# rsasaki0109/lidarslam_ros2

Hardware: AMD Instinct MI355X
Metric: scan registrations/sec (30k-pt scan vs 10-frame submap) (higher is better)
Workload: dtype f32; 1 GPU; cfg2: single NDT align(), 30000-pt VLP-32 scan (vg 0.2) vs 10-frame submap (vg 0.1), ndt_resolution 5.0, DIRECT7, max_iterations 30, transformation_epsilon 0; 1018 different scans (stream of 64); target_points=661519, voxels_valid=643, derivative_passes_last_scan=242, parallelism=1 registration stream per GPU x1, collective=none (one rank)

## Files before the change

### include/lidarslam_reg.h

```cpp
#ifndef LIDARSLAM_REG_H
#define LIDARSLAM_REG_H

#include <stddef.h>
#include <stdint.h>

#ifdef __cplusplus
extern "C" {
#endif

typedef struct lsr_handle_s* lsr_handle;

typedef enum lsr_status {
  LSR_OK = 0,
  LSR_ERR_INVALID_ARGUMENT = -1,
  LSR_ERR_NO_DEVICE = -2,
  LSR_ERR_HIP = -3,
  LSR_ERR_NO_TARGET = -4,
  LSR_ERR_NO_SOURCE = -5,
  LSR_ERR_NOT_IMPLEMENTED = -6,
  LSR_ERR_INDEX_OVERFLOW = -7,
  LSR_ERR_TOO_FEW_POINTS = -8
} lsr_status;

typedef enum lsr_method { LSR_METHOD_NDT = 0, LSR_METHOD_GICP = 1 } lsr_method;
// ... 6 lines not shown
  LSR_STEP_SIZE = 2,
  LSR_OUTLIER_RATIO = 3,
  LSR_MAX_CORRESPONDENCE_DISTANCE = 4,
  LSR_ROTATION_EPSILON = 5,
  LSR_EUCLIDEAN_FITNESS_EPSILON = 6,
  LSR_GICP_EPSILON = 7,
  LSR_MAP_ASSEMBLY_MS = 8,
  LSR_MAX_ITERATIONS = 32,
  LSR_NEIGHBORHOOD = 33,
  LSR_NUM_THREADS = 34,
  LSR_K_CORRESPONDENCES = 35,
  LSR_MAX_INNER_ITERATIONS = 36,
  LSR_RANSAC_ITERATIONS = 37,
  LSR_HESSIAN_D1_SIGN = 38,
  LSR_PROFILE = 39,
  LSR_NDT_WORKGROUP = 40,
  LSR_NDT_TABLE_MODE = 41,
  LSR_GRID_BUILDER = 42,
  LSR_WAIT_MODE = 43,
  LSR_NDT_QUAD = 44,
  LSR_VOXEL_FILTER_FORM = 46,
  LSR_NDT_SPLIT = 47,
  LSR_TARGET_PREPARED = 48,
  LSR_MAP_ASSEMBLY_FORM = 49
} lsr_key;

typedef struct lsr_result {
  int32_t converged;
  int32_t iterations;
  double score;
  int32_t n_evaluations;
  int32_t n_correspondences;
  double gpu_ms;
} lsr_result;

typedef struct lsr_profile {
  double deriv_ms_total;
  int64_t deriv_launches;
  int64_t deriv_points;
  int64_t deriv_pairs;
} lsr_profile;

const char* lsr_version(void);
const char* lsr_status_string(int status);
const char* lsr_last_error(void);
int lsr_device_count(int* count);

int lsr_create(int method, int device_id, void* stream, lsr_handle* out);
int lsr_destroy(lsr_handle h);

int lsr_set_f64(lsr_handle h, int key, double value);
int lsr_set_i32(lsr_handle h, int key, int value);
int lsr_get_f64(lsr_handle h, int key, double* value);
int lsr_get_i32(lsr_handle h, int key, int* value);

int lsr_set_input_target(lsr_handle h, const void* pts, size_t stride_bytes, size_t n);
int lsr_set_input_target_device(lsr_handle h, const void* dev_pts, size_t stride_bytes, size_t n);
int lsr_set_input_target_batch(lsr_handle* handles, int count, const void* const* clouds, const size_t* counts,
                               size_t stride_bytes, int on_device);
int lsr_wait_stream(lsr_handle h, void* producer_stream);
int lsr_set_input_target_frames(lsr_handle h, int n_frames, const void* const* frames, const size_t* counts, size_t stride_bytes,
                                const float* poses16, int on_device);
int lsr_set_input_target_frames_filtered(lsr_handle h, int n_frames, const void* const* frames, const size_t* counts,
// ... 128 lines not shown
```

### lidarslam_ros2_amd/_capi.py

```python
from __future__ import annotations

import ctypes as C
import os

_HERE = os.path.dirname(os.path.abspath(__file__))
LIB_PATH = os.path.join(_HERE, os.environ.get("LSR_LIB_NAME", "liblidarslam_reg.so"))

OK = 0
METHOD_NDT, METHOD_GICP = 0, 1
KDTREE, DIRECT26, DIRECT7, DIRECT1 = 0, 1, 2, 3
(RESOLUTION, TRANSFORMATION_EPSILON, STEP_SIZE, OUTLIER_RATIO, MAX_CORRESPONDENCE_DISTANCE, ROTATION_EPSILON,
 EUCLIDEAN_FITNESS_EPSILON, GICP_EPSILON, MAP_ASSEMBLY_MS) = range(9)
(MAX_ITERATIONS, NEIGHBORHOOD, NUM_THREADS, K_CORRESPONDENCES, MAX_INNER_ITERATIONS, RANSAC_ITERATIONS,
 HESSIAN_D1_SIGN, PROFILE, NDT_WORKGROUP, NDT_TABLE_MODE, GRID_BUILDER, WAIT_MODE, NDT_QUAD, _UNASSIGNED_45, VOXEL_FILTER_FORM, NDT_SPLIT, TARGET_PREPARED,
 MAP_ASSEMBLY_FORM) = range(32, 50)

EXPORTED_SYMBOLS = [
    "lsr_version", "lsr_status_string", "lsr_last_error", "lsr_device_count", "lsr_create", "lsr_destroy",
    "lsr_set_f64", "lsr_set_i32", "lsr_get_f64", "lsr_get_i32", "lsr_set_input_target", "lsr_set_input_target_device",
    "lsr_set_input_target_frames", "lsr_set_input_source", "lsr_set_input_source_device", "lsr_set_input_source_filtered", "lsr_set_input_source_frontend", "lsr_voxel_grid_filter",
    "lsr_share_target", "lsr_wait_stream", "lsr_align", "lsr_align_batch",
    "lsr_get_final_transformation", "lsr_has_converged", "lsr_get_fitness_score", "lsr_search_loop", "lsr_ndt_grid_info",
    "lsr_ndt_grid_dump", "lsr_ndt_grid_centroids", "lsr_ndt_derivatives", "lsr_ndt_derivatives_pairs", "lsr_gicp_covariances", "lsr_nearest_neighbors", "lsr_get_profile",
    "lsr_debug_angle_tables", "lsr_set_input_source_pc2", "lsr_get_source_pc2", "lsr_voxel_grid_filter_pc2", "lsr_shard_range", "lsr_comm_unique_id", "lsr_comm_create", "lsr_comm_destroy", "lsr_align_batch_sharded",
    "lsr_shard_plan", "lsr_align_batch_planned", "lsr_align_fitness_batch",
    "lsr_set_input_target_batch", "lsr_set_input_source_batch", "lsr_get_fitness_score_batch", "lsr_set_input_target_bcast", "lsr_get_source_pc2_device",
    "lsr_comm_all_gather_records", "lsr_set_input_target_frames_filtered", "lsr_prepare_target", "lsr_gicp_linearize",
    "lsr_imu_reset", "lsr_imu_push", "lsr_imu_receive", "lsr_imu_info", "lsr_deskew_pc2", "lsr_deskew_trace",
    "lsr_assemble_map",
]


class Result(C.Structure):
    _fields_ = [("converged", C.c_int32), ("iterations", C.c_int32), ("score", C.c_double),
                ("n_evaluations", C.c_int32), ("n_correspondences", C.c_int32), ("gpu_ms", C.c_double)]


class Profile(C.Structure):
    _fields_ = [("deriv_ms_total", C.c_double), ("deriv_launches", C.c_int64), ("deriv_points", C.c_int64),
                ("deriv_pairs", C.c_int64)]


class SubMap(C.Structure):
    _fields_ = [("position", C.c_double * 3), ("orientation", C.c_double * 4), ("distance", C.c_double),
                ("cloud", C.c_void_p), ("n_points", C.c_size_t)]


class LoopParams(C.Structure):
    _fields_ = [("threshold_loop_closure_score", C.c_double), ("distance_loop_closure", C.c_double),
                ("range_of_searching_loop_closure", C.c_double), ("search_submap_num", C.c_int),
                ("voxel_leaf_size", C.c_float), ("top_k", C.c_int), ("reserved", C.c_int)]


class LoopEdge(C.Structure):
    _fields_ = [("id_from", C.c_int), ("id_to", C.c_int), ("accepted", C.c_int), ("converged", C.c_int),
                ("iterations", C.c_int), ("n_target_points", C.c_int), ("candidate_distance", C.c_double),
                ("fitness_score", C.c_double), ("relative_pose", C.c_double * 16), ("final_transformation", C.c_float * 16)]


class Pc2Layout(C.Structure):
    _fields_ = [("point_step", C.c_uint32), ("offset_x", C.c_uint32), ("offset_y", C.c_uint32), ("offset_z", C.c_uint32),
                ("offset_intensity", C.c_int32)]

# ... 115 lines not shown
```

### lidarslam_ros2_amd/csrc/capi.hip

```cpp
#include <algorithm>
#include <chrono>
#include <functional>
#include <limits>
#include <cmath>
#include <cstdlib>
#include <mutex>
#include <numeric>
#include <thread>

#include "handle.hpp"

namespace lsr {
static thread_local std::string g_last_error;
void set_last_error(const std::string& s) { g_last_error = s; }
}

using namespace lsr;

namespace {

#define LSR_CHECK_HANDLE(h)                      \
  if (!(h)) {                                    \
    set_last_error("null handle");               \
    return LSR_ERR_INVALID_ARGUMENT;             \
// ... 569 lines not shown
  if (eager && !st) st = eager_dispatch(true);
  if (eager) {
    (void)hipEventRecord(lead->side_ev, lead->side_stream);
    for (int b = 0; b < B; b++) {
      if (!eager_sent[b]) continue;
      double v = 0;
      const int fst = nn_fitness_end(hs[b]->scratch, lead->side_stream, &v);
      if (fst && !st) st = fst;
      if (!fst) fitness_out[b] = v;
    }
  }
  if (prefetched || eager) {
    if (hipEventSynchronize(lead->side_ev) != hipSuccess && !st) { set_last_error("side-stream work of the candidate set failed"); st = LSR_ERR_HIP; }
    if (st && prefetched) for (int b = 0; b < B; b++) if (hs[b]->target) hs[b]->target->has_hash = false;
  }
  if (st) return st;
  const double ms = std::chrono::duration<double, std::milli>(std::chrono::steady_clock::now() - t0).count();
  const NdtMailbox* M = lead->mailbox.p;
  if (lead->profile) {
    LSR_HIP(hipEventRecord(lead->ev1, lead->stream));
    LSR_HIP(hipEventSynchronize(lead->ev1));
    float ev_ms = 0.f;
    LSR_HIP(hipEventElapsedTime(&ev_ms, lead->ev0, lead->ev1));
    int passes = 0;
    lead->prof.deriv_pairs = 0;
    for (int b = 0; b < B; b++) {
      passes = std::max(passes, M[b].n_passes);
      lead->prof.deriv_pairs += (int64_t)M[b].last_pairs;
    }
    lead->prof.deriv_ms_total += ev_ms;
    lead->prof.deriv_launches += passes;
    lead->prof.deriv_points += (int64_t)passes * pts;
  }
  for (int b = 0; b < B; b++) {
    lsr_handle h = hs[b];
    std::memcpy(h->final_T, M[b].final_T, sizeof(float) * 16);
    h->converged = M[b].converged;
    if (finals) std::memcpy(finals + 16 * b, M[b].final_T, sizeof(float) * 16);
    if (results) {
      results[b].converged = M[b].converged;
      results[b].iterations = M[b].nr_iterations;
      results[b].score = M[b].trans_probability;
      results[b].n_evaluations = M[b].n_evals;
      results[b].n_correspondences = (int)M[b].last_pairs;
      results[b].gpu_ms = ms;
    }
  }
  return LSR_OK;
}

}

extern "C" {

// ... 154 lines not shown
      if (v < 3 || v > GICP_MAX_K) { set_last_error("k_correspondences out of range"); return LSR_ERR_INVALID_ARGUMENT; }
      h->gicp.k = v; h->source_cov_valid = false; if (h->target) h->target->has_cov = false; return LSR_OK;
    case LSR_MAX_INNER_ITERATIONS: h->gicp.max_inner = v; return LSR_OK;
    case LSR_RANSAC_ITERATIONS: h->ransac_iterations = v; return LSR_OK;
    case LSR_HESSIAN_D1_SIGN: h->ndt.d1_sign = (v >= 0) ? 1 : -1; return LSR_OK;
    case LSR_PROFILE: h->profile = v ? 1 : 0; return LSR_OK;
    case LSR_NDT_WORKGROUP:
      if (v == 256) {
        static bool warned = false;
        if (!warned) { warned = true; fprintf(stderr, "[lidarslam_reg] LSR_NDT_WORKGROUP = 256 is a geometry of an earlier kernel: using the automatic choice (0)\n"); }
        h->ndt_threads = 0; return LSR_OK;
      }
      if (v != 0 && v != 64 && v != 128 && v != 512 && v != 1024) { set_last_error("NDT workgroup key must be 0 (auto), 64 / 128 (quad kernel: points) or 512 / 1024 (lane kernel: threads)"); return LSR_ERR_INVALID_ARGUMENT; }
      h->ndt_threads = v; return LSR_OK;
    case LSR_NDT_TABLE_MODE:
      if (v < -1 || v > 2) { set_last_error("NDT table mode must be in -1 .. 2: -1 (auto), 0 dense, 1 compact, 2 LDS"); return LSR_ERR_INVALID_ARGUMENT; }
      h->ndt_table_mode = v; return LSR_OK;
    case LSR_NDT_QUAD:
      if (v < -1 || v > 1) { set_last_error("NDT quad mode must be -1 (auto), 0 or 1"); return LSR_ERR_INVALID_ARGUMENT; }
      h->ndt_quad = v; return LSR_OK;
    case LSR_NDT_SPLIT:
      if (v < -1 || v > 1) { set_last_error("NDT split mode must be -1 (auto), 0 or 1"); return LSR_ERR_INVALID_ARGUMENT; }
      h->ndt_split = v; return LSR_OK;
    case LSR_GRID_BUILDER:
      if (v < 0 || v > 1) { set_last_error("grid builder must be 0 (auto) or 1 (radix-sort builder)"); return LSR_ERR_INVALID_ARGUMENT; }
      h->scratch.force_sort_path = (v == 1);
      if (h->target) h->target->has_grid = h->target->has_centroids = false;
      return LSR_OK;
    case LSR_WAIT_MODE:
      if (v < 0 || v > 2) { set_last_error("wait mode must be 0 (spin), 1 (yield) or 2 (sleep)"); return LSR_ERR_INVALID_ARGUMENT; }
      h->scratch.wait_mode = v; return LSR_OK;
    default: set_last_error("unknown i32 key"); return LSR_ERR_INVALID_ARGUMENT;
  }
}

int lsr_get_i32(lsr_handle h, int key, int* v) {
  LSR_CHECK_HANDLE(h);
  if (!v) return LSR_ERR_INVALID_ARGUMENT;
  switch (key) {
    case LSR_MAX_ITERATIONS: *v = (h->method == LSR_METHOD_NDT) ? h->ndt.max_iterations : h->gicp.max_iterations; return LSR_OK;
    case LSR_NEIGHBORHOOD: *v = h->ndt.neighborhood; return LSR_OK;
    case LSR_NUM_THREADS: *v = h->num_threads; return LSR_OK;
    case LSR_K_CORRESPONDENCES: *v = h->gicp.k; return LSR_OK;
    case LSR_MAX_INNER_ITERATIONS: *v = h->gicp.max_inner; return LSR_OK;
    case LSR_RANSAC_ITERATIONS: *v = h->ransac_iterations; return LSR_OK;
    case LSR_HESSIAN_D1_SIGN: *v = h->ndt.d1_sign; return LSR_OK;
    case LSR_PROFILE: *v = h->profile; return LSR_OK;
    case LSR_NDT_WORKGROUP: *v = h->ndt_threads; return LSR_OK;
    case LSR_NDT_TABLE_MODE: *v = h->ndt_table_mode; return LSR_OK;
    case LSR_NDT_QUAD: *v = h->ndt_quad; return LSR_OK;
    case LSR_NDT_SPLIT: *v = h->ndt_split; return LSR_OK;
    case LSR_GRID_BUILDER: *v = h->scratch.force_sort_path ? 1 : 0; return LSR_OK;
    case LSR_WAIT_MODE: *v = h->scratch.wait_mode; return LSR_OK;
    case LSR_VOXEL_FILTER_FORM: *v = h->scratch.vg_form; return LSR_OK;
    case LSR_MAP_ASSEMBLY_FORM: *v = h->map_form; return LSR_OK;
    case LSR_TARGET_PREPARED:
      if (h->method == LSR_METHOD_GICP) *v = gicp_target_prepared(h) ? 1 : 0;
      else *v = (h->target && h->target->n > 0 && h->target->has_grid && h->target->grid_leaf == (float)h->ndt.resolution &&
                 (h->ndt.neighborhood != LSR_KDTREE || h->target->has_centroids || h->target->grid.ncells == 0)) ? 1 : 0;
      return LSR_OK;
    default: set_last_error("unknown i32 key"); return LSR_ERR_INVALID_ARGUMENT;
  }
}

static int set_target_impl(lsr_handle h, const void* pts, size_t stride, size_t n, bool on_device) {
  LSR_CHECK_HANDLE(h);
  if (h->method == LSR_METHOD_NDT) {
    lsr_handle one[1] = {h};
    const void* cloud[1] = {pts};
    const size_t count[1] = {n};
    return lsr_set_input_target_batch(one, 1, cloud, count, stride, on_device ? 1 : 0);
  }
  auto t = fresh_target(h);
  int st = upload_cloud(h, pts, stride, n, on_device, t->cloud);
// ... 1020 lines not shown
  if (grad) for (int i = 0; i < 6; i++) grad[i] = S.g[i];
  if (hess) for (int i = 0; i < 36; i++) hess[i] = compute_hessian ? S.H[i] : 0.0;
  if (pairs) *pairs = S.last_pairs;
  return LSR_OK;
}

int lsr_gicp_covariances(lsr_handle h, int which, double* cov) {
  LSR_CHECK_HANDLE(h);
  if (!cov) return LSR_ERR_INVALID_ARGUMENT;
  return gicp_get_covariances(h, which, cov);
}

int lsr_gicp_linearize(lsr_handle h, const float* guess16, const float* trans16, int use_seeds, float* out, int32_t* nn_idx,
                       int32_t* valid, double* M6, float* q, double* x6, float* T12, double* dR27, int32_t* m, double* sums28) {
  LSR_CHECK_HANDLE(h);
  if (h->method != LSR_METHOD_GICP) { set_last_error("lsr_gicp_linearize on an NDT object"); return LSR_ERR_INVALID_ARGUMENT; }
  const GicpLinearizeOut o{out, nn_idx, valid, M6, q, x6, T12, dR27, m, sums28};
  return gicp_linearize(h, guess16, trans16, use_seeds, o);
}

int lsr_get_profile(lsr_handle h, lsr_profile* out, int reset) {
  LSR_CHECK_HANDLE(h);
  if (out) *out = h->prof;
  if (reset) h->prof = lsr_profile{0, 0, 0, 0};
  return LSR_OK;
}

}
```

### lidarslam_ros2_amd/csrc/handle.hpp

```cpp
#pragma once
#include "common.hpp"
#include "deskew.hpp"
#include "gicp.hpp"
#include "ndt.hpp"
#include "nn.hpp"

namespace lsr {
struct StreamDep {
  hipEvent_t ev = nullptr;
  ~StreamDep() { if (ev) (void)hipEventDestroy(ev); }
};
}

struct lsr_handle_s {
  using NdtParamsHost = lsr::NdtParamsHost; using GicpParamsHost = lsr::GicpParamsHost; using TargetData = lsr::TargetData;
  using DeviceCloud = lsr::DeviceCloud; using HashGridDev = lsr::HashGridDev; using BuildScratch = lsr::BuildScratch;
  using NdtState = lsr::NdtState; using NdtProblem = lsr::NdtProblem; using GicpWorkspace = lsr::GicpWorkspace;
  template <typename T> using DevBuf = lsr::DevBuf<T>;
  template <typename T> using PinBuf = lsr::PinBuf<T>;
  int method = LSR_METHOD_NDT;
  int device = 0;
  hipStream_t stream = nullptr;
  bool own_stream = false;
  hipEvent_t ev0 = nullptr, ev1 = nullptr;
// ... 39 lines not shown
  const NdtState* h_state_dev = nullptr;
  const NdtProblem* h_prob_dev = nullptr;
  PinBuf<lsr::NdtMailbox> mailbox;
  lsr::NdtMailbox* d_mailbox = nullptr;
  unsigned int align_token = 0;
  DevBuf<float> d_T16;
  DevBuf<float> d_poses;
  DevBuf<lsr::FrameSlot> d_frames;
  PinBuf<lsr::FrameSlot> h_frames;
  DevBuf<lsr::MapSlot> d_map_slots;
  PinBuf<lsr::MapSlot> h_map_slots;
  DevBuf<unsigned char> map_out;
  int map_form = 0;
  double map_ms = 0.0;

  GicpWorkspace gicp_ws;

  lsr::DeskewState deskew;

  std::vector<std::unique_ptr<lsr_handle_s>> aux;

  float final_T[16] = {1, 0, 0, 0, 0, 1, 0, 0, 0, 0, 1, 0, 0, 0, 0, 1};
  int converged = 0;
  lsr_profile prof = {0, 0, 0, 0};
};
```

### lidarslam_ros2_amd/csrc/ndt.hip

```cpp
#include "ndt.hpp"

#include <cmath>
#include <cstdlib>
#include <type_traits>

#include "grid_device.hpp"
#include "ndt_point.hpp"
#include "sort.hpp"

namespace lsr {

namespace {

__host__ __device__ inline void angle_tables(const double* p, bool with_hessian, int d1_sign, float* jang, float* hang) {
  double cx, cy, cz, sx, sy, sz;
  if (fabs(p[3]) < 10e-5) { cx = 1.0; sx = 0.0; } else { cx = cos(p[3]); sx = sin(p[3]); }
  if (fabs(p[4]) < 10e-5) { cy = 1.0; sy = 0.0; } else { cy = cos(p[4]); sy = sin(p[4]); }
  if (fabs(p[5]) < 10e-5) { cz = 1.0; sz = 0.0; } else { cz = cos(p[5]); sz = sin(p[5]); }
  jang[0] = (float)(-sx * sz + cx * sy * cz); jang[1] = (float)(-sx * cz - cx * sy * sz); jang[2] = (float)(-cx * cy);
  jang[3] = (float)(cx * sz + sx * sy * cz);  jang[4] = (float)(cx * cz - sx * sy * sz);  jang[5] = (float)(-sx * cy);
  jang[6] = (float)(-sy * cz);                jang[7] = (float)(sy * sz);                 jang[8] = (float)(cy);
  jang[9] = (float)(sx * cy * cz);            jang[10] = (float)(-sx * cy * sz);          jang[11] = (float)(sx * sy);
  jang[12] = (float)(-cx * cy * cz);          jang[13] = (float)(cx * cy * sz);           jang[14] = (float)(-cx * sy);
  jang[15] = (float)(-cy * sz);               jang[16] = (float)(-cy * cz);               jang[17] = 0.f;
// ... 33 lines not shown
  float s1 = sinf(res[0]), c1 = cosf(res[0]);
  res[2] = atan2f(s1 * c(2, 0) - c1 * c(1, 0), c1 * c(1, 1) - s1 * c(2, 1));
  res[0] = -res[0]; res[1] = -res[1]; res[2] = -res[2];
}

}

void ndt_gauss_constants(double resolution, double outlier_ratio, double* d1, double* d2) {
  double c1 = 10 * (1 - outlier_ratio);
  double c2 = outlier_ratio / pow(resolution, 3);
  double d3 = -log(c2);
  *d1 = -log(c1 + c2) - d3;
  *d2 = -2 * log((-log(c1 * exp(-0.5) + c2) - d3) / *d1);
}

void ndt_fill_align_constants(NdtState& st, const NdtParamsHost& prm, int n_points) {
  ndt_gauss_constants(prm.resolution, prm.outlier_ratio, &st.d1, &st.d2);
  st.step_max = prm.step_size;
  st.step_min = prm.trans_eps / 2;
  st.eps = prm.trans_eps;
  st.max_iter = prm.max_iterations;
  st.n_points = n_points;
  st.d1_sign = prm.d1_sign;
}

void ndt_fill_initial_state(NdtState& st, const float* guess16 , const NdtParamsHost& prm, int n_points) {
  std::memset(&st, 0, sizeof(st));
  ndt_fill_align_constants(st, prm, n_points);
  float I16[16] = {1, 0, 0, 0, 0, 1, 0, 0, 0, 0, 1, 0, 0, 0, 0, 1};
  const float* G = guess16 ? guess16 : I16;
  std::memcpy(st.final_T, G, sizeof(I16));
  st.T[0] = G[0]; st.T[1] = G[4]; st.T[2] = G[8];  st.T[3] = G[12];
  st.T[4] = G[1]; st.T[5] = G[5]; st.T[6] = G[9];  st.T[7] = G[13];
  st.T[8] = G[2]; st.T[9] = G[6]; st.T[10] = G[10]; st.T[11] = G[14];
  float e[3];
  euler012_f(G, e);
  st.p[0] = G[12]; st.p[1] = G[13]; st.p[2] = G[14];
  st.p[3] = e[0]; st.p[4] = e[1]; st.p[5] = e[2];
  for (int i = 0; i < 6; i++) st.x_t[i] = st.p[i];
  angle_tables(st.p, true, st.d1_sign, st.jang, st.hang);
  st.want_hessian = 1;
  st.phase = PH_INIT;
  st.done = 0;
}

void ndt_fill_diag_state(NdtState& st, const double* p6, const float* T16, int compute_hessian, const NdtParamsHost& prm,
// ... 256 lines not shown
  } else if (lane == 6) {
    f[0] = 1.0;
    f[7] = 0.0;
  }
  wave_lds_fence();
  const bool with_hang = (mode & 2) != 0;
  if (lane < 24 || with_hang) {
    double val = angle_entry_value(ent_a, f);
    if (lane == 24 + 20 && S->d1_sign < 0) val = -val;
    if (lane < 24) S->jang[lane] = (float)val; else S->hang[lane - 24] = (float)val;
  }
  if (with_hang && lane < 8) S->hang[40 + lane] = (float)angle_entry_value(ent_b, f);
  if (lane == 63) {
    float* T = S->T;
    compose_R12(cs_f[0], cs_f[1], cs_f[2], cs_f[3], cs_f[4], cs_f[5], T);
    T[3] = (float)S->x_t[0]; T[7] = (float)S->x_t[1]; T[11] = (float)S->x_t[2];
    T12_to_colmajor16(T, S->final_T);
  }
  if (lane == 0) S->pad1 = 0;
  wave_lds_fence();
}

enum CtlNext : int { CTL_DONE = 0, CTL_NEWTON_BEGIN = 1, CTL_NEWTON_END = 2 };

__device__ __forceinline__ int ndt_controller_mt(LdsState* S, const LdsDouble* sums) {
  const double mu = 1.e-4, nu = 0.9;
  const int max_step_iterations = 10;
  double sv[8];
#pragma unroll
  for (int k = 0; k < 8; k++) sv[k] = sums[k];
  const int phase = S->phase;
  const bool had_hessian = S->want_hessian != 0;
  const int n_evals = S->n_evals + (phase == PH_MT_LAST ? 2 : 1);
  const int n_passes = S->n_passes + 1;
  if (phase == PH_INIT || phase == PH_MT_HESS || phase == PH_DIAG) {
    S->n_evals = n_evals;
    S->n_passes = n_passes;
    S->last_pairs = sv[7];
    if (phase != PH_MT_HESS) {
      S->score = sv[0];
#pragma unroll
      for (int i = 0; i < 6; i++) S->g[i] = sv[1 + i];
    }
    if (phase == PH_DIAG) {
      if (had_hessian) {
        double hu[21];
#pragma unroll
        for (int k = 0; k < 21; k++) hu[k] = sums[8 + k];
        int k = 0;
#pragma unroll
// ... 222 lines not shown
    unsigned long long* _r = (unsigned long long*)&g_lsr_timing[(810 + ((hess) ? 1 : 0)) * 32]; \
    atomicAdd(&_r[0], 1ull); atomicAdd(&_r[1], (unsigned long long)(_p_t1 - _p_t0)); atomicAdd(&_r[2], (unsigned long long)(_p_t2 - _p_t7)); \
    atomicAdd(&_r[3], (unsigned long long)(_t3 - _p_t2)); atomicAdd(&_r[4], (unsigned long long)(_c3 - _p_c0)); atomicAdd(&_r[5], (unsigned long long)(_t3 - _p_t0)); \
  }
#else
#define LSR_STAMP(k)
#define LSR_STAMP_T(k, t)
#define LSR_SPAN_BEGIN(seq)
#define LSR_SPAN_END(seq)
#define LSR_CTL_BEGIN(L)
#define LSR_CTL_END(col)
#define LSR_PASS_BEGIN()
#define LSR_PASS_MARK(var)
#define LSR_PASS_END(hess)
#endif

__device__ __forceinline__ int uniform_i(int v) { return __builtin_amdgcn_readfirstlane(v); }
__device__ __forceinline__ float uniform_f(float v) { return __int_as_float(__builtin_amdgcn_readfirstlane(__float_as_int(v))); }
__device__ __forceinline__ double uniform_d(double v) {
  const int lo = __builtin_amdgcn_readfirstlane(__double2loint(v)), hi = __builtin_amdgcn_readfirstlane(__double2hiint(v));
  return __hiloint2double(hi, lo);
}

template <int CTRL>
__device__ __forceinline__ double dpp_quad_xor(double v) {
  int lo = __double2loint(v), hi = __double2hiint(v);
  lo = __builtin_amdgcn_update_dpp(0, lo, CTRL, 0xF, 0xF, true);
  hi = __builtin_amdgcn_update_dpp(0, hi, CTRL, 0xF, 0xF, true);
  return __hiloint2double(hi, lo);
}

template <int NOFF>
struct Offsets;
template <>
struct Offsets<1> {
  static __device__ __forceinline__ void get(int o, int& dx, int& dy, int& dz) { dx = dy = dz = 0; }
};
template <>
struct Offsets<7> {
  static __device__ __forceinline__ void get(int o, int& dx, int& dy, int& dz) {
    dx = (o == 1) - (o == 2);
    dy = (o == 3) - (o == 4);
    dz = (o == 5) - (o == 6);
  }
};
template <>
// ... 40 lines not shown
  t += (double)a.y; t += (double)a.z; t += (double)a.w;
  t += (double)b.x; t += (double)b.y; t += (double)b.z; t += (double)b.w;
  t += (double)c.x; t += (double)c.y; t += (double)c.z; t += (double)c.w;
  t += (double)d.x; t += (double)d.y; t += (double)d.z; t += (double)d.w;
  t += dpp_quad_xor<0xB1>(t);
  t += dpp_quad_xor<0x4E>(t);
  return t;
}
__device__ __forceinline__ void add_piece_lds(unsigned long long* ibin, const int v, const int k, const double t) {
  bool poison;
  const int m = piece(t, k, &poison);
  if (m != 0) atomicAdd(&ibin[k * 32 + v], (unsigned long long)(long long)m);
  if (poison && k == 0) atomicAdd(&ibin[31], 1ull);
}
}


__device__ __forceinline__ float dpp_quad_sum(float v) {
  v += __int_as_float(__builtin_amdgcn_update_dpp(0, __float_as_int(v), 0xB1, 0xF, 0xF, true));
  v += __int_as_float(__builtin_amdgcn_update_dpp(0, __float_as_int(v), 0x4E, 0xF, 0xF, true));
  return v;
}

template <int NOFF, int TAB, int PTS, bool KD = false>
__global__ __launch_bounds__(4 * PTS) void ndt_eval_quad_kernel(const NdtProblem P, const int seq) {
  constexpr int THREADS = 4 * PTS;
  constexpr int PITCH_PT = PTS + 8, PITCH_O = PTS + 4;
  constexpr int NT = (NOFF + 3) / 4;
  static_assert(PTS % 64 == 0, "a workgroup batch is a whole number of canonical chunks");
  if ((int)blockIdx.x >= P.nblocks) return;
  const int tid = threadIdx.x, ql = tid & 3, pq = tid >> 2;
  LSR_STAMP(0)
  LSR_STAMP_T(9, THREADS - 64)
  LSR_PASS_BEGIN()
  LSR_SPAN_BEGIN(seq)

  __shared__ float s_pt[14][PITCH_PT];
  __shared__ __attribute__((aligned(16))) float s_o[29][PITCH_O];
  __shared__ double s_bin[NDT_NBINS][32];
  __shared__ unsigned long long s_ibin[NDT_NBINS * 32];
  __shared__ double s_sum[NDT_NRED];
  __shared__ double s_lu[8][2];
  constexpr int STATE_Q = (int)(sizeof(NdtState) / 16);
  __shared__ uint4 s_state_q[STATE_Q];
  unsigned int* s_state = reinterpret_cast<unsigned int*>(s_state_q);
  extern __shared__ uint4 s_table[];

  const NdtState* __restrict__ Sin = P.st + (seq & 1);
// ... 39 lines not shown
      uint4* gq = reinterpret_cast<uint4*>(Sout);
      if (tid < STATE_Q) gq[tid] = s_state_q[tid];
    }
    return;
  }
  if (TAB == NDT_TAB_LDS) {
    const int nchunks = P.lds_bytes >> 10;
    const unsigned char* img = reinterpret_cast<const unsigned char*>(P.lds_image) + (size_t)(tid & 63) * 16;
    unsigned char* dst = reinterpret_cast<unsigned char*>(s_table);
    if (tid >= 64)
      for (int c = (tid >> 6) - 1; c < nchunks; c += THREADS / 64 - 1)
        __builtin_amdgcn_global_load_lds((const __attribute__((address_space(1))) void*)(img + (size_t)c * 1024),
                                         (__attribute__((address_space(3))) void*)(dst + (size_t)c * 1024), 16, 0, 0);
  }
  if (tid < 64) {
    if (seq > 0) {
      if (tid < NDT_NRED) {
        double t = (((s_bin[4][tid] + s_bin[3][tid]) + s_bin[2][tid]) + s_bin[1][tid]) + s_bin[0][tid];
        if (s_bin[0][31] != 0.0 || s_bin[1][31] != 0.0) t = __longlong_as_double(0x7FF8000000000000ll);
        s_sum[tid] = t;
      }
      wave_lds_fence();
      LSR_STAMP(6)
      LSR_CTL_BEGIN(L)
      ndt_controller_wave0(L, (const LdsDouble*)s_sum);
      wave_lds_fence();
      LSR_CTL_END(0)
      LSR_STAMP(5)
      build_request_wave0(reinterpret_cast<NdtState*>(s_state), &s_lu[0][0], reinterpret_cast<float*>(&s_lu[4][0]), ang_entry, ang_entry_b);
      LSR_CTL_END(2)
      LSR_STAMP(4)
    }
    if (blockIdx.x == 0) {
      uint4* gq = reinterpret_cast<uint4*>(Sout);
      gq[tid] = s_state_q[tid];
      if (tid + 64 < STATE_Q) gq[tid + 64] = s_state_q[tid + 64];
    }
  }
  __syncthreads();
  if (uniform_i(L->done)) {
    if (P.mailbox != nullptr && blockIdx.x == 0 && tid == 0) {
      NdtMailbox* mb = P.mailbox;
#pragma unroll
      for (int k = 0; k < 16; k++) mb->final_T[k] = L->final_T[k];
      mb->converged = L->converged;
      mb->nr_iterations = L->nr_iterations;
      mb->n_evals = L->n_evals;
      mb->n_passes = L->n_passes;
      mb->trans_probability = L->trans_probability;
      mb->last_pairs = L->last_pairs;
      __threadfence_system();
      __hip_atomic_store(&mb->done, (unsigned int)L->token, __ATOMIC_RELEASE, __HIP_MEMORY_SCOPE_SYSTEM);
    }
    return;
  }
  if (blockIdx.x == 0) {
    uint4* zb = reinterpret_cast<uint4*>(P.bins + (size_t)((seq + 1) % NDT_NBANKS) * NDT_BANK_WORDS);
    for (int k = tid; k < NDT_BANK_WORDS / 2; k += THREADS) zb[k] = make_uint4(0u, 0u, 0u, 0u);
  }
  LSR_STAMP(7)
  LSR_PASS_MARK(_p_t7)

  const int form = uniform_i(L->want_hessian);
  const bool hess = form != NDT_PASS_GRAD;
  const bool fused = form == NDT_PASS_FUSED;
  const double d1d = uniform_d(L->d1);
  const float d2 = uniform_f((float)L->d2);
  float T[12];
#pragma unroll
  for (int k = 0; k < 12; k++) T[k] = uniform_f(L->T[k]);
  const float leaf = P.leaf;
// ... 259 lines not shown
    if (blockIdx.x == 0 && seq > 0) {
      uint4* gq = reinterpret_cast<uint4*>(Sout);
      if (tid < STATE_Q) gq[tid] = s_state_q[tid];
    }
    return;
  }
  if (TAB == NDT_TAB_LDS) {
    const int nchunks = P.lds_bytes >> 10;
    const unsigned char* img = reinterpret_cast<const unsigned char*>(P.lds_image) + (size_t)lane * 16;
    unsigned char* dst = reinterpret_cast<unsigned char*>(s_table);
    if (tid >= 64)
      for (int c = wave - 1; c < nchunks; c += NWAVES - 1)
        __builtin_amdgcn_global_load_lds((const __attribute__((address_space(1))) void*)(img + (size_t)c * 1024),
                                         (__attribute__((address_space(3))) void*)(dst + (size_t)c * 1024), 16, 0, 0);
  }
  if (tid < 64) {
    if (seq > 0) {
      if (tid < NDT_NRED) {
        double t = (((s_bin[4][tid] + s_bin[3][tid]) + s_bin[2][tid]) + s_bin[1][tid]) + s_bin[0][tid];
        if (s_bin[0][31] != 0.0 || s_bin[1][31] != 0.0) t = __longlong_as_double(0x7FF8000000000000ll);
        s_sum[tid] = t;
      }
      wave_lds_fence();
      ndt_controller_wave0(L, (const LdsDouble*)s_sum);
      wave_lds_fence();
      build_request_wave0(reinterpret_cast<NdtState*>(s_state), &s_lu[0][0], reinterpret_cast<float*>(&s_lu[4][0]), ang_entry, ang_entry_b);
    }
    if (blockIdx.x == 0) {
      uint4* gq = reinterpret_cast<uint4*>(Sout);
      gq[tid] = s_state_q[tid];
      if (tid + 64 < STATE_Q) gq[tid + 64] = s_state_q[tid + 64];
    }
  }
  __syncthreads();
  if (uniform_i(L->done)) {
    if (P.mailbox != nullptr && blockIdx.x == 0 && tid == 0) {
      NdtMailbox* mb = P.mailbox;
#pragma unroll
      for (int k = 0; k < 16; k++) mb->final_T[k] = L->final_T[k];
      mb->converged = L->converged;
      mb->nr_iterations = L->nr_iterations;
      mb->n_evals = L->n_evals;
      mb->n_passes = L->n_passes;
      mb->trans_probability = L->trans_probability;
      mb->last_pairs = L->last_pairs;
      __threadfence_system();
      __hip_atomic_store(&mb->done, (unsigned int)L->token, __ATOMIC_RELEASE, __HIP_MEMORY_SCOPE_SYSTEM);
    }
    return;
  }
  if (blockIdx.x == 0) {
    uint4* zb = reinterpret_cast<uint4*>(P.bins + (size_t)((seq + 1) % NDT_NBANKS) * NDT_BANK_WORDS);
    for (int k = tid; k < NDT_BANK_WORDS / 2; k += THREADS) zb[k] = make_uint4(0u, 0u, 0u, 0u);
  }

  const int form = uniform_i(L->want_hessian);
  const bool hess = form != NDT_PASS_GRAD;
  const bool fused = form == NDT_PASS_FUSED;
  const double d1d = uniform_d(L->d1);
  const float d2 = uniform_f((float)L->d2);
  float T[12];
#pragma unroll
  for (int k = 0; k < 12; k++) T[k] = uniform_f(L->T[k]);
  const float leaf = P.leaf;
  const int mb0 = P.min_b[0], mb1 = P.min_b[1], mb2 = P.min_b[2];
  const int xb0 = P.max_b[0], xb1 = P.max_b[1], xb2 = P.max_b[2];
// ... 377 lines not shown
```

### lidarslam_ros2_amd/csrc/ndt.hpp

```cpp
#pragma once
#include "common.hpp"

namespace lsr {

enum NdtPhase : int {
  PH_INIT = 0,
  PH_MT_FIRST = 1,
  PH_MT_TRIAL = 2,
  PH_MT_HESS = 3,
  PH_DIAG = 4,
  PH_MT_LAST = 5
};

enum NdtPassForm : int {
  NDT_PASS_GRAD = 0,
  NDT_PASS_HESS = 1,
  NDT_PASS_FUSED = 2
};

constexpr int NDT_NRED = 32;
constexpr int NDT_NRED_GRAD = 8;
constexpr int NDT_LANE_THREADS = 512;
constexpr int NDT_MAX_BLOCKS = 1024;
constexpr int ndt_lane_tile_bytes(int threads) { return (threads / 64) * 16 * 68 * 4; }
// ... 17 lines not shown

struct NdtState {
  float T[12];
  float jang[24];
  float hang[48];
  int want_hessian;
  int done;
  int phase;
  int d1_sign;
  double d1, d2;
  double step_max, step_min, eps;
  int max_iter, n_points;
  double p[6], x_t[6], dir[6];
  double score, g[6], H[36];
  int nr_iterations, converged;
  double phi_0, d_phi_0, a_l, f_l, g_l, a_u, f_u, g_u, a_t;
  int open_interval, interval_converged, step_iterations;
  int token;
  float final_T[16];
  double trans_probability;
  double last_pairs;
  int n_evals, pad1;
  int n_passes;
  int pad2[3];
};
static_assert(sizeof(NdtState) % 16 == 0 && sizeof(NdtState) <= 128 * 16, "NdtState travels as at most 128 uint4");

struct NdtMailbox {
  unsigned long long progress;
  unsigned int done;
  int converged, nr_iterations, n_evals;
  double trans_probability, last_pairs;
  float final_T[16];
  int n_passes;
};

struct NdtProblem {
  const float* sx;
  const float* sy;
  const float* sz;
  int n;
  int nblocks;
  const int* cell_slot;
  const float4* rec;
  int min_b[3];
  int max_b[3];
  int mul1, mul2;
  float leaf;
  int lds_map_bytes;
  const uint4* lds_image;
  int lds_bytes;
  long long* bins;
  NdtState* st;
  NdtMailbox* mailbox;
  const float4* centroid;
  float radius2;
};

struct NdtParamsHost {
  double resolution = 1.0, step_size = 0.1, outlier_ratio = 0.55, trans_eps = 0.1;
  int max_iterations = 35;
  int neighborhood = LSR_DIRECT7;
  int d1_sign = 1;
};

void ndt_gauss_constants(double resolution, double outlier_ratio, double* d1, double* d2);

int cloud_bbox(const DeviceCloud& cloud, float* mn, float* mx, unsigned int* n_finite, BuildScratch& sc, hipStream_t stream);
int cloud_bbox_begin(const DeviceCloud& cloud, BuildScratch& sc, hipStream_t stream);
int cloud_bbox_end(const DeviceCloud& cloud, float* mn, float* mx, unsigned int* n_finite, BuildScratch& sc, hipStream_t stream);

int ndt_build_grid(DeviceCloud& cloud, float leaf, VoxelGridDev& grid, BuildScratch& sc, hipStream_t stream);
int ndt_build_grid_end(VoxelGridDev& grid, BuildScratch& sc, hipStream_t stream);
int ndt_build_centroids(const DeviceCloud& cloud, VoxelGridDev& grid, BuildScratch& sc, hipStream_t stream);

struct NdtLaunchCfg {
  int batch = 1;
  int max_blocks = 1;
  int neighborhood = LSR_DIRECT7;
  int tab = NDT_TAB_DENSE;
  int threads = NDT_LANE_THREADS;
  int lds_bytes = 0;
  int split = 0;
  int quad = 0;
};
constexpr int NDT_QUAD_THREADS = 512;
// ... 45 lines not shown
```

### lidarslam_ros2_amd/registration.py

```python
from __future__ import annotations

import ctypes as C
from typing import Optional, Sequence

import numpy as np

from . import _capi as capi

DIRECT7, DIRECT1, DIRECT26, KDTREE = capi.DIRECT7, capi.DIRECT1, capi.DIRECT26, capi.KDTREE
PC2_XYZI = (32, (0, 4, 8, 16))


def _is_torch_cuda(x) -> bool:
    return hasattr(x, "is_cuda") and bool(x.is_cuda)


def _cloud_args(cloud, reg=None):
    if _is_torch_cuda(cloud):
        import torch

        t = cloud
        if t.dtype != torch.float32 or t.dim() != 2 or t.shape[1] < 3:
            raise ValueError("device cloud must be float32 of shape (n, c>=3)")
        if not t.is_contiguous():
# ... 381 lines not shown
        idx = np.zeros(self._n_source, np.int32)
        d2 = np.zeros(self._n_source, np.float32)
        t = _mat_to_col16(T) if T is not None else None
        capi.check(self._lib.lsr_nearest_neighbors(self._h, t.ctypes.data_as(C.POINTER(C.c_float)) if t is not None else None,
                                                   idx.ctypes.data_as(C.POINTER(C.c_int32)),
                                                   d2.ctypes.data_as(C.POINTER(C.c_float))), "nearestNeighbors")
        return idx, d2

    def setTuning(self, workgroup: Optional[int] = None, table_mode: Optional[int] = None, grid_builder: Optional[int] = None,
                  wait_mode: Optional[int] = None, quad: Optional[int] = None, split: Optional[int] = None):
        if workgroup is not None:
            self._seti(capi.NDT_WORKGROUP, workgroup, "setTuning(workgroup)")
        if table_mode is not None:
            self._seti(capi.NDT_TABLE_MODE, table_mode, "setTuning(table_mode)")
        if grid_builder is not None:
            self._seti(capi.GRID_BUILDER, grid_builder, "setTuning(grid_builder)")
        if wait_mode is not None:
            self._seti(capi.WAIT_MODE, wait_mode, "setTuning(wait_mode)")
        if quad is not None:
            self._seti(capi.NDT_QUAD, quad, "setTuning(quad)")
        if split is not None:
            self._seti(capi.NDT_SPLIT, split, "setTuning(split)")

    def setProfiling(self, on: bool):
        self._seti(capi.PROFILE, 1 if on else 0, "setProfiling")

    def getProfile(self, reset: bool = False) -> dict:
        p = capi.Profile()
        capi.check(self._lib.lsr_get_profile(self._h, C.byref(p), 1 if reset else 0), "getProfile")
        return dict(deriv_ms_total=p.deriv_ms_total, deriv_launches=p.deriv_launches, deriv_points=p.deriv_points,
                    deriv_pairs=p.deriv_pairs)


class NormalDistributionsTransform(Registration):

    _method = capi.METHOD_NDT

    def setResolution(self, res: float):
        self._setf(capi.RESOLUTION, res, "setResolution")

    def getResolution(self) -> float:
        return self._getf(capi.RESOLUTION)

    def setStepSize(self, s: float):
        self._setf(capi.STEP_SIZE, s, "setStepSize")

    def getStepSize(self) -> float:
        return self._getf(capi.STEP_SIZE)

    def setOulierRatio(self, r: float):
        self._setf(capi.OUTLIER_RATIO, r, "setOulierRatio")

    setOutlierRatio = setOulierRatio

# ... 175 lines not shown
```

Baseline: 461.0 registrations/s.

## Reuse gradient pass results when the line-search request repeats unchanged

After the controller builds the next evaluation request in a gradient-only line-search trial, the kernel now checks whether the 36-word request (transform plus angle Jacobian) matches the one just evaluated. If it does, the controller keeps stepping on the existing sums instead of launching another derivative pass over the scan. This skips redundant full passes during More-Thuente trials. Alongside, the quad kernel gets an amdgpu_waves_per_eu occupancy hint chosen per neighborhood and table mode. Reuse is on by default, can be toggled through a new key, and is counted in the profile.

After: 717.8 registrations/s, median of 6. +55.7%, better.

```diff
diff --git a/include/lidarslam_reg.h b/include/lidarslam_reg.h
--- a/include/lidarslam_reg.h
+++ b/include/lidarslam_reg.h
@@ -52,7 +52,8 @@
   LSR_VOXEL_FILTER_FORM = 46,
   LSR_NDT_SPLIT = 47,
   LSR_TARGET_PREPARED = 48,
-  LSR_MAP_ASSEMBLY_FORM = 49
+  LSR_MAP_ASSEMBLY_FORM = 49,
+  LSR_NDT_PASS_REUSE = 50
 } lsr_key;
 
 typedef struct lsr_result {
@@ -69,6 +70,7 @@
   int64_t deriv_launches;
   int64_t deriv_points;
   int64_t deriv_pairs;
+  int64_t deriv_reused;
 } lsr_profile;
 
 const char* lsr_version(void);
diff --git a/lidarslam_ros2_amd/_capi.py b/lidarslam_ros2_amd/_capi.py
--- a/lidarslam_ros2_amd/_capi.py
+++ b/lidarslam_ros2_amd/_capi.py
@@ -13,7 +13,7 @@
  EUCLIDEAN_FITNESS_EPSILON, GICP_EPSILON, MAP_ASSEMBLY_MS) = range(9)
 (MAX_ITERATIONS, NEIGHBORHOOD, NUM_THREADS, K_CORRESPONDENCES, MAX_INNER_ITERATIONS, RANSAC_ITERATIONS,
  HESSIAN_D1_SIGN, PROFILE, NDT_WORKGROUP, NDT_TABLE_MODE, GRID_BUILDER, WAIT_MODE, NDT_QUAD, _UNASSIGNED_45, VOXEL_FILTER_FORM, NDT_SPLIT, TARGET_PREPARED,
- MAP_ASSEMBLY_FORM) = range(32, 50)
+ MAP_ASSEMBLY_FORM, NDT_PASS_REUSE) = range(32, 51)
 
 EXPORTED_SYMBOLS = [
     "lsr_version", "lsr_status_string", "lsr_last_error", "lsr_device_count", "lsr_create", "lsr_destroy",
@@ -38,7 +38,7 @@
 
 class Profile(C.Structure):
     _fields_ = [("deriv_ms_total", C.c_double), ("deriv_launches", C.c_int64), ("deriv_points", C.c_int64),
-                ("deriv_pairs", C.c_int64)]
+                ("deriv_pairs", C.c_int64), ("deriv_reused", C.c_int64)]
 
 
 class SubMap(C.Structure):
diff --git a/lidarslam_ros2_amd/csrc/capi.hip b/lidarslam_ros2_amd/csrc/capi.hip
--- a/lidarslam_ros2_amd/csrc/capi.hip
+++ b/lidarslam_ros2_amd/csrc/capi.hip
@@ -615,14 +615,15 @@
     LSR_HIP(hipEventSynchronize(lead->ev1));
     float ev_ms = 0.f;
     LSR_HIP(hipEventElapsedTime(&ev_ms, lead->ev0, lead->ev1));
-    int passes = 0;
+    int passes = 0, reused = 0;
     lead->prof.deriv_pairs = 0;
     for (int b = 0; b < B; b++) {
-      passes = std::max(passes, M[b].n_passes);
+      if (M[b].n_passes > passes) { passes = M[b].n_passes; reused = M[b].n_reused; }
       lead->prof.deriv_pairs += (int64_t)M[b].last_pairs;
     }
     lead->prof.deriv_ms_total += ev_ms;
     lead->prof.deriv_launches += passes;
+    lead->prof.deriv_reused += reused;
     lead->prof.deriv_points += (int64_t)passes * pts;
   }
   for (int b = 0; b < B; b++) {
@@ -823,6 +824,7 @@
     case LSR_NDT_SPLIT:
       if (v < -1 || v > 1) { set_last_error("NDT split mode must be -1 (auto), 0 or 1"); return LSR_ERR_INVALID_ARGUMENT; }
       h->ndt_split = v; return LSR_OK;
+    case LSR_NDT_PASS_REUSE: h->ndt.pass_reuse = v ? 1 : 0; return LSR_OK;
     case LSR_GRID_BUILDER:
       if (v < 0 || v > 1) { set_last_error("grid builder must be 0 (auto) or 1 (radix-sort builder)"); return LSR_ERR_INVALID_ARGUMENT; }
       h->scratch.force_sort_path = (v == 1);
@@ -851,6 +853,7 @@
     case LSR_NDT_TABLE_MODE: *v = h->ndt_table_mode; return LSR_OK;
     case LSR_NDT_QUAD: *v = h->ndt_quad; return LSR_OK;
     case LSR_NDT_SPLIT: *v = h->ndt_split; return LSR_OK;
+    case LSR_NDT_PASS_REUSE: *v = h->ndt.pass_reuse; return LSR_OK;
     case LSR_GRID_BUILDER: *v = h->scratch.force_sort_path ? 1 : 0; return LSR_OK;
     case LSR_WAIT_MODE: *v = h->scratch.wait_mode; return LSR_OK;
     case LSR_VOXEL_FILTER_FORM: *v = h->scratch.vg_form; return LSR_OK;
@@ -1917,8 +1920,8 @@
 int lsr_get_profile(lsr_handle h, lsr_profile* out, int reset) {
   LSR_CHECK_HANDLE(h);
   if (out) *out = h->prof;
-  if (reset) h->prof = lsr_profile{0, 0, 0, 0};
-  return LSR_OK;
-}
-
-}
+  if (reset) h->prof = lsr_profile{0, 0, 0, 0, 0};
+  return LSR_OK;
+}
+
+}
diff --git a/lidarslam_ros2_amd/csrc/handle.hpp b/lidarslam_ros2_amd/csrc/handle.hpp
--- a/lidarslam_ros2_amd/csrc/handle.hpp
+++ b/lidarslam_ros2_amd/csrc/handle.hpp
@@ -85,5 +85,5 @@
 
   float final_T[16] = {1, 0, 0, 0, 0, 1, 0, 0, 0, 0, 1, 0, 0, 0, 0, 1};
   int converged = 0;
-  lsr_profile prof = {0, 0, 0, 0};
+  lsr_profile prof = {0, 0, 0, 0, 0};
 };
diff --git a/lidarslam_ros2_amd/csrc/ndt.hip b/lidarslam_ros2_amd/csrc/ndt.hip
--- a/lidarslam_ros2_amd/csrc/ndt.hip
+++ b/lidarslam_ros2_amd/csrc/ndt.hip
@@ -79,6 +79,7 @@
   st.max_iter = prm.max_iterations;
   st.n_points = n_points;
   st.d1_sign = prm.d1_sign;
+  st.reuse = prm.pass_reuse ? 1 : 0;
 }
 
 void ndt_fill_initial_state(NdtState& st, const float* guess16 , const NdtParamsHost& prm, int n_points) {
@@ -381,10 +382,11 @@
 }
 
 enum CtlNext : int { CTL_DONE = 0, CTL_NEWTON_BEGIN = 1, CTL_NEWTON_END = 2 };
+constexpr int NDT_MAX_STEP_ITERATIONS = 10;
 
 __device__ __forceinline__ int ndt_controller_mt(LdsState* S, const LdsDouble* sums) {
   const double mu = 1.e-4, nu = 0.9;
-  const int max_step_iterations = 10;
+  const int max_step_iterations = NDT_MAX_STEP_ITERATIONS;
   double sv[8];
 #pragma unroll
   for (int k = 0; k < 8; k++) sv[k] = sums[k];
@@ -653,6 +655,52 @@
   return __hiloint2double(hi, lo);
 }
 
+constexpr int NDT_REQUEST_WORDS = 36;
+static_assert(offsetof(NdtState, T) == 0 && offsetof(NdtState, jang) == 48 && offsetof(NdtState, hang) == 4 * NDT_REQUEST_WORDS,
+              "T and jang are the first 36 words of the state");
+typedef __attribute__((address_space(3))) unsigned int LdsWord;
+__device__ __forceinline__ bool ndt_request_repeats(LdsState* L, const LdsWord* s_state, const unsigned int kept) {
+  if (uniform_i(L->done) != 0 || uniform_i(L->phase) != PH_MT_TRIAL) return false;
+  const int lane = threadIdx.x;
+  const bool same = lane >= NDT_REQUEST_WORDS || s_state[lane] == kept;
+  return __builtin_amdgcn_ballot_w64(same) == ~0ull;
+}
+__device__ __attribute__((noinline)) void ndt_repeat_steps_wave0(LdsState* L, LdsWord* s_state, const LdsDouble* sums, LdsDouble* f ,
+                                                                 const unsigned int ent_a, const unsigned int ent_b, const unsigned int kept) {
+  const int lane = threadIdx.x;
+  for (int turn = 0; turn < NDT_MAX_STEP_ITERATIONS; turn++) {
+    int next = CTL_DONE;
+    if (lane == 0) {
+      L->n_reused = L->n_reused + 1;
+      next = ndt_controller_mt(L, sums);
+    }
+    if (__builtin_amdgcn_readfirstlane(next) != CTL_DONE) {
+      if (lane == 0) { L->trans_probability = L->score / (double)L->n_points; L->done = 1; }
+      wave_lds_fence();
+      return;
+    }
+    wave_lds_fence();
+    build_request_wave0((NdtState*)L, (double*)f, (float*)(f + 8), ent_a, ent_b);
+    if (!ndt_request_repeats(L, s_state, kept)) return;
+  }
+}
+__device__ __forceinline__ void ndt_head_wave0(LdsState* L, unsigned int* s_state, const LdsDouble* sums, double* f ,
+                                               const unsigned int ent_a, const unsigned int ent_b) {
+  const int lane = threadIdx.x;
+  const unsigned int kept = lane < NDT_REQUEST_WORDS ? s_state[lane] : 0u;
+  const bool reusable = uniform_i(L->reuse) != 0 && uniform_i(L->want_hessian) == NDT_PASS_GRAD;
+  LSR_CTL_BEGIN(L)
+  ndt_controller_wave0(L, sums);
+  wave_lds_fence();
+  LSR_CTL_END(0)
+  LSR_STAMP(5)
+  build_request_wave0(reinterpret_cast<NdtState*>(s_state), f, reinterpret_cast<float*>(f + 8), ent_a, ent_b);
+  LSR_CTL_END(2)
+  LSR_STAMP(4)
+  if (reusable && ndt_request_repeats(L, (const LdsWord*)s_state, kept))
+    ndt_repeat_steps_wave0(L, (LdsWord*)s_state, sums, (LdsDouble*)f, ent_a, ent_b, kept);
+}
+
 template <int CTRL>
 __device__ __forceinline__ double dpp_quad_xor(double v) {
   int lo = __double2loint(v), hi = __double2hiint(v);
@@ -739,8 +787,10 @@
   return v;
 }
 
+constexpr int ndt_quad_waves_per_simd(int noff, int tab, bool kd) { return noff < 27 ? 4 : ((kd && tab == NDT_TAB_DENSE) ? 2 : 3); }
 template <int NOFF, int TAB, int PTS, bool KD = false>
-__global__ __launch_bounds__(4 * PTS) void ndt_eval_quad_kernel(const NdtProblem P, const int seq) {
+__global__ __launch_bounds__(4 * PTS) __attribute__((amdgpu_waves_per_eu(ndt_quad_waves_per_simd(NOFF, TAB, KD))))
+void ndt_eval_quad_kernel(const NdtProblem P, const int seq) {
   constexpr int THREADS = 4 * PTS;
   constexpr int PITCH_PT = PTS + 8, PITCH_O = PTS + 4;
   constexpr int NT = (NOFF + 3) / 4;
@@ -826,14 +876,7 @@
       }
       wave_lds_fence();
       LSR_STAMP(6)
-      LSR_CTL_BEGIN(L)
-      ndt_controller_wave0(L, (const LdsDouble*)s_sum);
-      wave_lds_fence();
-      LSR_CTL_END(0)
-      LSR_STAMP(5)
-      build_request_wave0(reinterpret_cast<NdtState*>(s_state), &s_lu[0][0], reinterpret_cast<float*>(&s_lu[4][0]), ang_entry, ang_entry_b);
-      LSR_CTL_END(2)
-      LSR_STAMP(4)
+      ndt_head_wave0(L, s_state, (const LdsDouble*)s_sum, &s_lu[0][0], ang_entry, ang_entry_b);
     }
     if (blockIdx.x == 0) {
       uint4* gq = reinterpret_cast<uint4*>(Sout);
@@ -851,6 +894,7 @@
       mb->nr_iterations = L->nr_iterations;
       mb->n_evals = L->n_evals;
       mb->n_passes = L->n_passes;
+      mb->n_reused = L->n_reused;
       mb->trans_probability = L->trans_probability;
       mb->last_pairs = L->last_pairs;
       __threadfence_system();
@@ -1156,9 +1200,7 @@
         s_sum[tid] = t;
       }
       wave_lds_fence();
-      ndt_controller_wave0(L, (const LdsDouble*)s_sum);
-      wave_lds_fence();
-      build_request_wave0(reinterpret_cast<NdtState*>(s_state), &s_lu[0][0], reinterpret_cast<float*>(&s_lu[4][0]), ang_entry, ang_entry_b);
+      ndt_head_wave0(L, s_state, (const LdsDouble*)s_sum, &s_lu[0][0], ang_entry, ang_entry_b);
     }
     if (blockIdx.x == 0) {
       uint4* gq = reinterpret_cast<uint4*>(Sout);
@@ -1176,6 +1218,7 @@
       mb->nr_iterations = L->nr_iterations;
       mb->n_evals = L->n_evals;
       mb->n_passes = L->n_passes;
+      mb->n_reused = L->n_reused;
       mb->trans_probability = L->trans_probability;
       mb->last_pairs = L->last_pairs;
       __threadfence_system();
diff --git a/lidarslam_ros2_amd/csrc/ndt.hpp b/lidarslam_ros2_amd/csrc/ndt.hpp
--- a/lidarslam_ros2_amd/csrc/ndt.hpp
+++ b/lidarslam_ros2_amd/csrc/ndt.hpp
@@ -63,7 +63,9 @@
   double last_pairs;
   int n_evals, pad1;
   int n_passes;
-  int pad2[3];
+  int n_reused;
+  int reuse;
+  int pad2;
 };
 static_assert(sizeof(NdtState) % 16 == 0 && sizeof(NdtState) <= 128 * 16, "NdtState travels as at most 128 uint4");
 
@@ -74,6 +76,7 @@
   double trans_probability, last_pairs;
   float final_T[16];
   int n_passes;
+  int n_reused;
 };
 
 struct NdtProblem {
@@ -103,6 +106,7 @@
   int max_iterations = 35;
   int neighborhood = LSR_DIRECT7;
   int d1_sign = 1;
+  int pass_reuse = 1;
 };
 
 void ndt_gauss_constants(double resolution, double outlier_ratio, double* d1, double* d2);
diff --git a/lidarslam_ros2_amd/registration.py b/lidarslam_ros2_amd/registration.py
--- a/lidarslam_ros2_amd/registration.py
+++ b/lidarslam_ros2_amd/registration.py
@@ -427,6 +427,9 @@
         if split is not None:
             self._seti(capi.NDT_SPLIT, split, "setTuning(split)")
 
+    def setPassReuse(self, on: bool):
+        self._seti(capi.NDT_PASS_REUSE, 1 if on else 0, "setPassReuse")
+
     def setProfiling(self, on: bool):
         self._seti(capi.PROFILE, 1 if on else 0, "setProfiling")
 
@@ -434,7 +437,7 @@
         p = capi.Profile()
         capi.check(self._lib.lsr_get_profile(self._h, C.byref(p), 1 if reset else 0), "getProfile")
         return dict(deriv_ms_total=p.deriv_ms_total, deriv_launches=p.deriv_launches, deriv_points=p.deriv_points,
-                    deriv_pairs=p.deriv_pairs)
+                    deriv_pairs=p.deriv_pairs, deriv_reused=p.deriv_reused)
 
 
 class NormalDistributionsTransform(Registration):
```
